# jstac/sdfs_via_autodiff

Hardware: AMD Instinct MI355X
Metric: fixed-point iterations/sec (higher is better)
Workload: dtype f64

## Files before the change

include/sdfs_hip.h:

```cpp
#ifndef SDFS_HIP_H
#define SDFS_HIP_H

#include <stdint.h>

#ifdef __cplusplus
extern "C" {
#endif

typedef struct sdfs_handle sdfs_handle;

enum { SDFS_MODEL_SSY = 0, SDFS_MODEL_GCY = 1 };
enum { SDFS_ALGO_SA = 0, SDFS_ALGO_NEWTON = 1, SDFS_ALGO_ANDERSON = 2 };

enum {
  SDFS_OK = 0,
  SDFS_ERR_ARG = -1,
  SDFS_ERR_HIP = -2,
  SDFS_ERR_UNSUPPORTED = -3,
  SDFS_ERR_NUMERIC = -4
};

typedef struct sdfs_opts {
  double tol;
  int64_t max_iter;
// ... 136 lines not shown
int sdfs_set_t_f32(sdfs_handle* h, int on, double w_ref);

int sdfs_set_profiling(sdfs_handle* h, int on);
int sdfs_reset_counters(sdfs_handle* h);
int sdfs_get_counters(sdfs_handle* h, sdfs_counters* out);

int sdfs_debug_pow(const double* x_host, double y, double* out_host, int64_t n, int device_id);
int sdfs_debug_powy(const double* x_host, double y, double* out_host, int64_t n, int degree, int device_id);
int sdfs_debug_jvp_storage_dev(sdfs_handle* h, int krylov_f32, const double* w_dev, const void* v_dev, void* out_dev,
                               int minus_identity);

int sdfs_stream_copy_dev(sdfs_handle* h, const double* src_dev, double* dst_dev, int64_t n);

int sdfs_describe_plan(const sdfs_handle* h, char* buf, int64_t cap);

typedef struct sdfs_batch sdfs_batch;

enum { SDFS_BATCH_CONVERGED = 0, SDFS_BATCH_MAX_ITER = 1, SDFS_BATCH_NONFINITE = 2 };

int64_t sdfs_batch_lds_bytes(int model, int ndim, const int64_t* shapes);

int sdfs_batch_create(int model, int ndim, const int64_t* shapes, int64_t B, const double* params,
                      const double* const* arrays, const int64_t* array_sizes, int narrays, int device_id,
                      sdfs_batch** out);
void sdfs_batch_destroy(sdfs_batch* h);
const char* sdfs_batch_last_error(const sdfs_batch* h);
int sdfs_batch_set_stream(sdfs_batch* h, void* hip_stream, int use_own);
int sdfs_batch_synchronize(sdfs_batch* h);

int sdfs_batch_apply_T_dev(sdfs_batch* h, const double* w_dev, double* Tw_dev, double* resid_dev);
// ... 14 lines not shown
```

sdfs_via_autodiff_amd/_lib.py:

```python
import ctypes as C
import os

_HERE = os.path.dirname(os.path.abspath(__file__))
LIB_PATH = os.path.join(_HERE, os.environ.get("SDFS_LIB_NAME", "libsdfs_hip.so"))

SDFS_MODEL_SSY, SDFS_MODEL_GCY = 0, 1
SDFS_ALGO_SA, SDFS_ALGO_NEWTON, SDFS_ALGO_ANDERSON = 0, 1, 2
SDFS_ERR_ARG = -1
SDFS_ERR_UNSUPPORTED = -3
SDFS_ERR_NUMERIC = -4
SDFS_MAX_KERNELS = 16
SDFS_BATCH_CONVERGED, SDFS_BATCH_MAX_ITER, SDFS_BATCH_NONFINITE = 0, 1, 2


class SdfsError(RuntimeError):
    pass


class sdfs_opts(C.Structure):
    _fields_ = [("tol", C.c_double), ("max_iter", C.c_int64),
                ("inner_rtol", C.c_double), ("inner_atol", C.c_double),
                ("inner_max_iter", C.c_int64),
                ("history", C.c_int32), ("mixing_freq", C.c_int32),
                ("beta", C.c_double), ("ridge", C.c_double),
# ... 66 lines not shown
    "sdfs_unpack_blocks_sub": (C.c_int, [_P, _P, _P, _P, C.c_int64, C.c_int64, C.c_int64, C.c_int, C.POINTER(C.c_int64), C.c_int]),
    "sdfs_anderson_begin": (C.c_int, [_P, C.c_int64, C.c_int, _P, _P, C.c_double, C.c_int64, C.c_double, C.c_double, C.c_int]),
    "sdfs_anderson_gate": (C.c_int, [_P, C.POINTER(_P)]),
    "sdfs_anderson_step": (C.c_int, [_P, C.c_int, C.c_int64, _P, _P, _P]),
    "sdfs_anderson_state": (C.c_int, [_P, _P, _P, C.c_int64, C.c_int64]),
    "sdfs_set_krylov_f32": (C.c_int, [_P, C.c_int, C.c_double]),
    "sdfs_set_t_f32": (C.c_int, [_P, C.c_int, C.c_double]),
    "sdfs_set_profiling": (C.c_int, [_P, C.c_int]),
    "sdfs_reset_counters": (C.c_int, [_P]),
    "sdfs_get_counters": (C.c_int, [_P, C.POINTER(sdfs_counters)]),
    "sdfs_describe_plan": (C.c_int, [_P, C.c_char_p, C.c_int64]),
    "sdfs_stream_copy_dev": (C.c_int, [_P, _P, _P, C.c_int64]),
    "sdfs_debug_pow": (C.c_int, [_P, C.c_double, _P, C.c_int64, C.c_int]),
    "sdfs_debug_powy": (C.c_int, [_P, C.c_double, _P, C.c_int64, C.c_int, C.c_int]),
    "sdfs_debug_jvp_storage_dev": (C.c_int, [_P, C.c_int, _P, _P, _P, C.c_int]),
    "sdfs_batch_lds_bytes": (C.c_int64, [C.c_int, C.c_int, _I64]),
    "sdfs_batch_create": (C.c_int, [C.c_int, C.c_int, _I64, C.c_int64, _D, C.POINTER(_D), _I64, C.c_int, C.c_int,
                                    C.POINTER(_P)]),
    "sdfs_batch_destroy": (None, [_P]),
    "sdfs_batch_last_error": (C.c_char_p, [_P]),
    "sdfs_batch_set_stream": (C.c_int, [_P, _P, C.c_int]),
    "sdfs_batch_synchronize": (C.c_int, [_P]),
    "sdfs_batch_apply_T_dev": (C.c_int, [_P, _P, _P, _P]),
    "sdfs_batch_solve_dev": (C.c_int, [_P, C.POINTER(sdfs_opts), _P, _I64, _D, C.POINTER(C.c_int32)]),
    "sdfs_batch_newton_dev": (C.c_int, [_P, C.POINTER(sdfs_opts), _P, _I64, _I64, _D, C.POINTER(C.c_int32)]),
    "sdfs_batch_describe": (C.c_int, [_P, C.c_char_p, C.c_int64]),
}


def _load():
# ... 35 lines not shown
```

sdfs_via_autodiff_amd/csrc/f32_kernels.hpp:

```cpp
#pragma once
#include "fast_kernels.hpp"

namespace sdfs {

typedef float v4f __attribute__((ext_vector_type(4)));
typedef float v2f __attribute__((ext_vector_type(2)));

template <int N> struct MShape32 {
  static_assert(N == 16 || N == 20 || N == 24 || N == 32, "pair plan extents");
  static constexpr int NT = (N + 15) / 16;
  static constexpr int KT = N / 4;
};

template <int N> struct QFrag32 {
  float a[MShape32<N>::NT][MShape32<N>::KT];
  __device__ __forceinline__ void load(const double* __restrict__ Q, int lane) {
    using S = MShape32<N>;
    const int li = lane & 15, lk = lane >> 4;
#pragma unroll
    for (int t = 0; t < S::NT; ++t) {
      const int row = 16 * t + li;
#pragma unroll
      for (int kk = 0; kk < S::KT; ++kk) a[t][kk] = row < N ? (float)Q[(row < N ? row : 0) * N + 4 * kk + lk] : 0.f;
    }
  }
};

template <int N, int RS>
__device__ __forceinline__ void ctile32(float* __restrict__ col, const int lk, const QFrag32<N>& q) {
  using S = MShape32<N>;
  float b[S::KT];
  const float* const pr = col + lk * RS;
#pragma unroll
  for (int kk = 0; kk < S::KT; ++kk) b[kk] = pr[4 * kk * RS];
  v4f acc[S::NT];
#pragma unroll
  for (int t = 0; t < S::NT; ++t) acc[t] = (v4f){0.f, 0.f, 0.f, 0.f};
#pragma unroll
  for (int kk = 0; kk < S::KT; ++kk) {
// ... 275 lines not shown
```

sdfs_via_autodiff_amd/csrc/fast_kernels.hpp:

```cpp
#pragma once
#include <hip/hip_runtime.h>
#include <stdint.h>

#include <type_traits>

#include "anderson_step.hpp"
#include "pass_kernel.hpp"
#include "wave_reduce.hpp"

namespace sdfs {

enum SliceMode { S_TFIRST = 0, S_TFIRST_LIN = 1, S_JFIRST = 2, S_MID = 3, S_TFIRST32 = 4, S_NMODES = 5 };
enum LineMode { L_MID = 0, L_TLAST = 1, L_TLAST_LIN = 2, L_JLAST = 3, L_TFUSED = 4, L_NMODES = 5 };

template <int N> struct MShape {
  static_assert(N == 16 || N == 20 || N == 24 || N == 32, "pair plan extents");
  static constexpr int N16 = N == 32 ? 2 : 1;
  static constexpr int N4 = (N - 16 * N16) / 4;
  static constexpr int KT = N / 4;
  static constexpr int A16 = N16, A4 = N4 > 0 ? N4 : 1;
};

template <int N> struct QFrag {
  double a16[MShape<N>::A16][MShape<N>::KT];
  double a4[MShape<N>::A4][MShape<N>::KT];
  __device__ __forceinline__ void load(const double* __restrict__ Q, int lane) {
    using S = MShape<N>;
    const int li = lane & 15, lk = lane >> 4, l4 = lane & 3;
#pragma unroll
    for (int kk = 0; kk < S::KT; ++kk) {
#pragma unroll
      for (int t = 0; t < S::N16; ++t) a16[t][kk] = Q[(16 * t + li) * N + 4 * kk + lk];
#pragma unroll
      for (int t = 0; t < S::N4; ++t) a4[t][kk] = Q[(16 * S::N16 + 4 * t + l4) * N + 4 * kk + lk];
    }
  }
};

template <int N, int RS>
__device__ __forceinline__ void ctile(double* __restrict__ p, const QFrag<N>& q) {
  using S = MShape<N>;
  double b[S::KT];
#pragma unroll
  for (int kk = 0; kk < S::KT; ++kk) b[kk] = p[4 * kk * RS];
  v4d acc[S::A16];
  double d[S::A4];
#pragma unroll
  for (int t = 0; t < S::A16; ++t) acc[t] = (v4d){0.0, 0.0, 0.0, 0.0};
#pragma unroll
// ... 91 lines not shown
template <int N, int WV = 4, bool PAD20 = false, int GX = 0> struct SliceGeo {
  static constexpr int G = GX > 0 ? GX : (N == 32 ? 2 : (N == 24 ? 2 : 4));
  static constexpr int RS = (N == 20 && !PAD20) ? N : N + 2;
  static constexpr int LTILE = G * N * RS;
  static constexpr int TILE = G * N * N;
  static constexpr int UNITS = TILE / 2;
  static constexpr int EPT = (UNITS + 63) / 64;
  static constexpr int NCT = (G * N + 15) / 16;
  static constexpr int CPAD = NCT * 16 - G * N;
  static constexpr int WAVES = WV;
  static constexpr int UNITS4 = TILE / 4;
  static constexpr int EPT4 = (UNITS4 + 63) / 64;
  static_assert(CPAD <= 8, "the repeated columns lie inside the last column tile");
};

template <int N, int MODE, bool F32, int WV = 4, bool PAD20 = false, int GX = 0, int OCC = 3>
__global__ void __launch_bounds__(64 * WV, OCC)
slice_kernel(const SliceDesc P, const SliceIO io) {
  using Geo = SliceGeo<N, WV, PAD20, GX>;
  constexpr bool T32 = MODE == S_TFIRST32;
  constexpr bool POWP = MODE == S_TFIRST || MODE == S_TFIRST_LIN || T32;
  constexpr bool LIN = MODE == S_TFIRST_LIN;
  constexpr bool MULP = MODE == S_JFIRST;
  constexpr bool JV32 = F32 && MULP;
  static_assert(!T32 || !F32, "S_TFIRST32 is its own storage form");
  constexpr bool POWREG = MODE == S_TFIRST || T32;
  static_assert(!F32 || (MODE != S_TFIRST && MODE != S_MID), "plain T has no fp32 form");
  extern __shared__ double lds[];
  if (io.gate != nullptr) {
    const unsigned long long g = *io.gate;
    if (g <= (unsigned long long)__double_as_longlong(io.gate_tol)) return;
  }
  const int lane = threadIdx.x & 63;
  const int wave = __builtin_amdgcn_readfirstlane(threadIdx.x >> 6);
  if (io.zero != nullptr && blockIdx.x == 0 && threadIdx.x == 0) *io.zero = 0ULL;
  const long long tile = (long long)blockIdx.x * Geo::WAVES + wave;
  const long long s0 = tile * Geo::G;
  if (s0 >= P.nslices) return;
  const long long rem = (P.nslices - s0) * (N * N / 2);
  const int nvalid = rem < Geo::UNITS ? (int)rem : Geo::UNITS;
  double* const wl = lds + wave * Geo::LTILE;
  auto lofs = [](const int e) -> int { return Geo::RS == N ? e : (e / N) * Geo::RS + (e % N); };
  const long long gbase = s0 * (N * N);
  const unsigned lb = (unsigned)lane * 16u;

  if (JV32) {
    const int nvalid4 = nvalid / 2;
    const char* const inb = reinterpret_cast<const char*>(reinterpret_cast<const float*>(io.in) + gbase);
    const char* const auxb = reinterpret_cast<const char*>(reinterpret_cast<const float*>(io.aux_in) + gbase);
    float4 v[Geo::EPT4], c1v[Geo::EPT4];
#pragma unroll
    for (int k = 0; k < Geo::EPT4; ++k) {
      const int u = lane + 64 * k;
      if (u < nvalid4) {
        v[k] = *reinterpret_cast<const float4*>(inb + (lb + 1024u * k));
        c1v[k] = *reinterpret_cast<const float4*>(auxb + (lb + 1024u * k));
      } else {
        v[k] = make_float4(0.f, 0.f, 0.f, 0.f); c1v[k] = v[k];
      }
    }
#pragma unroll
    for (int k = 0; k < Geo::EPT4; ++k) {
      const int u = lane + 64 * k;
      if (Geo::UNITS4 % 64 == 0 || u < Geo::UNITS4) {
        *reinterpret_cast<double2*>(wl + lofs(4 * u)) = make_double2((double)v[k].x * (double)c1v[k].x, (double)v[k].y * (double)c1v[k].y);
        *reinterpret_cast<double2*>(wl + lofs(4 * u + 2)) = make_double2((double)v[k].z * (double)c1v[k].z, (double)v[k].w * (double)c1v[k].w);
      }
    }
  } else {
    const char* const inb = reinterpret_cast<const char*>(io.in + gbase);
    const char* const auxb = reinterpret_cast<const char*>(io.aux_in + gbase);
    double2 v[Geo::EPT];
    double2 c1v[MULP ? Geo::EPT : 1];
#pragma unroll
    for (int k = 0; k < Geo::EPT; ++k) {
      const int u = lane + 64 * k;
      if (u < nvalid) {
        v[k] = ldg_stream2(inb + (lb + 1024u * k));
        if (MULP) c1v[MULP ? k : 0] = ldg_stream2(auxb + (lb + 1024u * k));
      } else {
        v[k] = make_double2(1.0, 1.0);
        if (MULP) c1v[MULP ? k : 0] = make_double2(0.0, 0.0);
      }
    }
    PowK<true> PTr;
    if (POWREG) PTr.init(P.theta, lane);
    double t32s = 1.0;
    if (T32) { const PowLane PL0 = pow_lane_init(lane); t32s = t32_scale_of(P.t32_ref > 0.0 ? P.t32_ref : io.in[P.ref_off], P.theta, PL0, false); }
#pragma unroll
    for (int k = 0; k < Geo::EPT; ++k) {
      const int u = lane + 64 * k;
      if (MULP) { v[k].x *= c1v[MULP ? k : 0].x; v[k].y *= c1v[MULP ? k : 0].y; }
      if (POWREG) {
        const double xin[2] = {v[k].x, v[k].y};
        double xw[2];
        PTr.template run<2>(xin, xw);
        v[k] = T32 ? make_double2(xw[0] * t32s, xw[1] * t32s) : make_double2(xw[0], xw[1]);
      }
      if (Geo::UNITS % 64 == 0 || u < Geo::UNITS) *reinterpret_cast<double2*>(wl + lofs(2 * u)) = v[k];
    }
  }
  QFrag<N> qf;
  qf.load(P.Qf, lane);
  wave_lds_fence();
  if (POWP && !POWREG) {
    const PowLane PT = pow_lane_init(lane);
    double lin_scale = 1.0;
    if (LIN && F32) lin_scale = lin_scale_of(io.in[P.ref_off], P.theta, PT, false);
    const double t32_scale = T32 ? t32_scale_of(P.t32_ref > 0.0 ? P.t32_ref : io.in[P.ref_off], P.theta, PT, false) : 1.0;
    char* const auxo = LIN ? (F32 ? reinterpret_cast<char*>(reinterpret_cast<float*>(io.aux_out) + gbase)
                                  : reinterpret_cast<char*>(io.aux_out + gbase)) : nullptr;
#pragma unroll 1
    for (int k = 0; k < Geo::EPT; ++k) {
      const int u = lane + 64 * k;
      const bool in_tile = Geo::UNITS % 64 == 0 || u < Geo::UNITS;
      const int lo = in_tile ? lofs(2 * u) : 0;
      const double2 x2 = *reinterpret_cast<const double2*>(wl + lo);
      const double xin[2] = {in_tile ? x2.x : 1.0, in_tile ? x2.y : 1.0};
      double xw[2];
// ... 8 lines not shown
      }
    }
    wave_lds_fence();
  }

  const int li = lane & 15, lk = lane >> 4;
  {
    double* const p0 = wl + li * Geo::RS + lk;
#pragma unroll
    for (int ct = 0; ct < Geo::NCT; ++ct) {
      const bool rep = Geo::CPAD > 0 && ct == Geo::NCT - 1;
      ctile<N, 1>(p0 + (ct * 16 - ((rep && li >= 16 - Geo::CPAD) ? Geo::CPAD : 0)) * Geo::RS, qf);
    }
  }
  wave_lds_fence();
  {
    QFrag<N> qe;
    qe.load(P.Qe, lane);
#pragma unroll
    for (int ct = 0; ct < Geo::NCT; ++ct) {
      const bool rep = Geo::CPAD > 0 && ct == Geo::NCT - 1;
      const int c = 16 * ct + li - ((rep && li >= 16 - Geo::CPAD) ? Geo::CPAD : 0);
      const int g = c / N, f = c - g * N;
      ctile<N, Geo::RS>(wl + g * (N * Geo::RS) + f + lk * Geo::RS, qe);
    }
  }
  wave_lds_fence();
  if (JV32 || T32) {
    const int nvalid4 = nvalid / 2;
    char* const outb = reinterpret_cast<char*>(reinterpret_cast<float*>(io.out) + gbase);
#pragma unroll
    for (int k = 0; k < Geo::EPT4; ++k) {
      const int u = lane + 64 * k;
      if (u < nvalid4) {
        const double2 a = *reinterpret_cast<const double2*>(wl + lofs(4 * u)), b = *reinterpret_cast<const double2*>(wl + lofs(4 * u + 2));
        *reinterpret_cast<float4*>(outb + (lb + 1024u * k)) = make_float4((float)a.x, (float)a.y, (float)b.x, (float)b.y);
      }
    }
  } else {
    char* const outb = reinterpret_cast<char*>(io.out + gbase);
#pragma unroll
    for (int k = 0; k < Geo::EPT; ++k) {
// ... 1053 lines not shown
```

sdfs_via_autodiff_amd/csrc/pad_kernels.hpp:

```cpp
#pragma once
#include <hip/hip_runtime.h>
#include <stdint.h>

#include "fast_kernels.hpp"

#ifndef SDFS_PAD_SOCC16
#define SDFS_PAD_SOCC16 3
#endif
#ifndef SDFS_PAD_SOCC24
#define SDFS_PAD_SOCC24 3
#endif
#ifndef SDFS_PAD_SOCC32
#define SDFS_PAD_SOCC32 3
#endif
#ifndef SDFS_PAD_SOCC16_J
#define SDFS_PAD_SOCC16_J 3
#endif
#ifndef SDFS_PAD_LOCC_MID16
#define SDFS_PAD_LOCC_MID16 3
#endif
#ifndef SDFS_PAD_LOCC_MID24
#define SDFS_PAD_LOCC_MID24 3
#endif
#ifndef SDFS_PAD_LOCC_MID32
// ... 79 lines not shown
      if (MULP) c1v[MULP ? k : 0] = e < nval ? io.aux_in[gbase + e] : 0.0;
    }
  }
#pragma unroll
  for (int k = 0; k < (PAD_LT + 63) / 64; ++k)
    if (PAD_LT % 64 == 0 || lane + 64 * k < PAD_LT) wl[lane + 64 * k] = 0.0;
  int lo[PAD_EPL];
#pragma unroll
  for (int k = 0; k < PAD_EPL; ++k) {
    const unsigned e = (unsigned)EI(k);
    const unsigned s = (e * P.mxy) >> 20, r = e - s * (unsigned)nxy;
    const unsigned x = (r * P.my) >> 20, y = r - x * (unsigned)P.ny;
    lo[k] = (int)((s * (unsigned)NT + x) * (unsigned)PAD_RS + y);
  }
  QFrag<NT> qf;
  qf.load(P.Qy, lane);
  wave_lds_fence();
  if (POWP) {
    PowK<true> PT;
    PT.init(P.theta, lane);
#pragma unroll
    for (int k = 0; k < PAD_EPL; k += 2) {
      if (NT == 32 && (PAIR ? 128 * (k >> 1) : 64 * k) >= nval) break;
      const double xin[2] = {v[k], v[k + 1]};
      double xw[2];
      PT.template run<2>(xin, xw);
      if (LIN) {
        if (PAIR) {
          if (EI(k) < nval) *reinterpret_cast<v2d*>(io.aux_out + gbase + EI(k)) = (v2d){xw[0] / xin[0], xw[1] / xin[1]};
        } else {
          if (EI(k) < nval) io.aux_out[gbase + EI(k)] = xw[0] / xin[0];
// ... 7 lines not shown
  for (int k = 0; k < PAD_EPL; ++k) {
    if (MULP) v[k] *= c1v[MULP ? k : 0];
    if (EI(k) < nval) wl[lo[k]] = v[k];
  }
  wave_lds_fence();
  const int li = lane & 15, lk = lane >> 4;
  constexpr int NCT = PAD_G * NT / 16;
  {
    double* const p0 = wl + li * PAD_RS + lk;
#pragma unroll
    for (int ct = 0; ct < NCT; ++ct) ctile<NT, 1>(p0 + ct * 16 * PAD_RS, qf);
  }
  wave_lds_fence();
  {
    QFrag<NT> qe;
    qe.load(P.Qx, lane);
#pragma unroll
    for (int ct = 0; ct < NCT; ++ct) {
      const int c = 16 * ct + li;
      const int g = c / NT, f = c - g * NT;
      ctile<NT, PAD_RS>(wl + g * (NT * PAD_RS) + f + lk * PAD_RS, qe);
    }
  }
  wave_lds_fence();
  if (PAIR) {
#pragma unroll
    for (int k = 0; k < PAD_EPL; k += 2)
      if (EI(k) < nval) *reinterpret_cast<v2d*>(io.out + gbase + EI(k)) = (v2d){wl[lo[k]], wl[lo[k + 1]]};
  } else {
#pragma unroll
    for (int k = 0; k < PAD_EPL; ++k)
// ... 64 lines not shown
  {
    double2 v[EPT];
#pragma unroll
    for (int k = 0; k < EPT; ++k) {
      int x, y; bool rok; long long off;
      unit_of(k, x, y, rok, off);
      v[k] = ld2(inb + off, pk0 && rok, pk1 && rok);
      if ((CES || MULE) && need_old) s1[(CES || MULE) ? k : 0] = ld2(oldb + off, pk0 && rok, pk1 && rok);
    }
#pragma unroll
    for (int k = 0; k < EPT; ++k)
      if (!Geo::PARTIAL || tid + B * k < Geo::UNITS) *reinterpret_cast<double2*>(lds + 2 * (tid + B * k)) = v[k];
  }
  {
    QFrag<NT> q;
    q.load(P.Qx, lane);
    __syncthreads();
    {
      double* const p0 = lds + li + lk * Geo::LX;
#pragma unroll
      for (int j = 0; j < (Geo::NCT + Geo::W - 1) / Geo::W; ++j)
        if (Geo::NCT % Geo::W == 0 || wave + j * Geo::W < Geo::NCT) ctile<NT, Geo::LX>(p0 + (wave + j * Geo::W) * 16, q);
    }
    q.load(P.Qy, lane);
    __syncthreads();
    {
      constexpr int XPT = 16 / R;
      double* const p0 = lds + (li / R) * Geo::LX + (li % R) + lk * R;
#pragma unroll
      for (int j = 0; j < (Geo::NCT + Geo::W - 1) / Geo::W; ++j)
        if (Geo::NCT % Geo::W == 0 || wave + j * Geo::W < Geo::NCT) ctile<NT, R>(p0 + (wave + j * Geo::W) * XPT * Geo::LX, q);
    }
    __syncthreads();
  }
  double* const outb = io.out + tbase;
  double rmax = 0.0, dot_yv = 0.0, dot_yy = 0.0;
  bool rnan = false;
  if (CES) {
    PowK<false> PT;
// ... 120 lines not shown
```

sdfs_via_autodiff_amd/csrc/sdfs_api.hip:

```cpp
#include <hip/hip_runtime.h>

#include <algorithm>
#include <cmath>
#include <cstdarg>
#include <cstdio>
#include <cstdlib>
#include <cstring>
#include <limits>
#include <map>
#include <mutex>
#include <string>
#include <type_traits>
#include <vector>

#include "../../include/sdfs_hip.h"
#include "pass_kernel.hpp"
#include "fast_kernels.hpp"
#include "stream_kernels.hpp"
#include "f32_kernels.hpp"
#include "pad_kernels.hpp"
#include "cont_kernel.hpp"
#include "dense_kernel.hpp"
#include "vec_kernels.hpp"
#include "krylov_kernels.hpp"
// ... 6 lines not shown
using namespace sdfs;

namespace {

constexpr int MAXD = 6;
constexpr int SCHED_WORDS = TK_WORDS;

thread_local std::string g_create_error;

struct AxisInfo {
  int n = 1;
  int nloc = 1;
  int off = 0;
  const double* Q = nullptr;
  const double* Qt = nullptr;
  const double* Qp = nullptr;
  const double* Qtp = nullptr;
  const double* Qpad[4] = {nullptr, nullptr, nullptr, nullptr};
  const double* Qtpad[4] = {nullptr, nullptr, nullptr, nullptr};
  int qs[MAXD] = {0, 0, 0, 0, 0, 0};
  long long qcount = 0;
  int a3s = 0;
  char name[8] = "";
};

struct Pass {
  PassDesc d;
  int block = 256;
  bool vec2 = false;
  bool vec4 = false;
// ... 683 lines not shown

std::vector<int> pair_order(int D) {
  std::vector<int> pairs = {D - 2};
  for (int a = 0; a <= D - 4; a += 2) pairs.push_back(a);
  return pairs;
}

void make_slice_pass(sdfs_handle* h, const int* shp, FastPass& P) {
  const int D = h->ndim;
  long long stride[MAXD], nloc = 1;
  for (int a = D - 1; a >= 0; --a) { stride[a] = nloc; nloc *= shp[a]; }
  const int n = shp[D - 1];
  P.line = false; P.n = n; P.ax0 = D - 2; P.ax1 = D - 1;
  memset(&P.sd, 0, sizeof P.sd);
  P.sd.nslices = nloc / ((long long)n * n);
  P.sd.Qf = h->ax[D - 1].Q; P.sd.Qe = h->ax[D - 2].Q; P.sd.theta = h->theta;
  for (int c = D - 1; c >= 0; --c) P.sd.ref_off += (long long)(shp[c] / 2) * stride[c];
  P.q_bytes = 2 * 8.0 * n * n; P.flops = 2.0 * (double)nloc * 2 * n;
  P.label = std::string("slices[") + h->ax[D - 2].name + "," + h->ax[D - 1].name + "|wave-private " +
            std::to_string(slice_tile_slices(n, S_TFIRST)) + "x" + std::to_string(n) + "x" + std::to_string(n) + "]";
}

int make_line_pass(sdfs_handle* h, const int* shp, const int* off, int a, bool tables, FastPass& P) {
  const int D = h->ndim;
  long long stride[MAXD], nloc = 1;
  for (int c = D - 1; c >= 0; --c) { stride[c] = nloc; nloc *= shp[c]; }
  const int n = shp[a];
  P.line = true; P.n = n; P.ax0 = a; P.ax1 = a + 1;
  memset(&P.ld, 0, sizeof P.ld);
  LineDesc& L = P.ld;
  L.lrest = stride[a + 1];
  if (L.lrest % 2 != 0) return 1;
  L.nchunks = (int)((L.lrest + LINE_R - 1) / LINE_R);
  L.nouter = nloc / ((long long)n * n * L.lrest);
  L.ntiles = L.nouter * L.nchunks;
  if (L.ntiles >= (1LL << 31) || (long long)n * n * L.lrest * 8 >= (1LL << 32)) return 1;
  L.Qx = h->ax[a].Q; L.Qy = h->ax[a + 1].Q;
  L.inv_theta = 1.0 / h->theta; L.beta = h->beta; L.theta = h->theta;
  L.cbt = (double)powl((long double)h->beta, (long double)h->theta);
  L.a3x = h->ax[a].a3s; L.a3y = h->ax[a + 1].a3s;
  for (int c = D - 1; c >= 0; --c) L.ref_off += (long long)(shp[c] / 2) * stride[c];
  L.cached_out = 8.0 * (double)nloc <= 192.0 * 1024 * 1024 ? 1 : 0;
  P.q_bytes = 2 * 8.0 * n * n; P.flops = 2.0 * (double)nloc * 2 * n;
  P.label = std::string("lines[") + h->ax[a].name + "," + h->ax[a + 1].name + "|" + std::to_string(n) + "x" +
            std::to_string(n) + "x16 tile]";
  if (!tables) return 0;
  std::vector<int> outv, restv;
  int *od = nullptr, *rd = nullptr;
  int rc;
  if ((rc = a3_index_tables(h, shp, off, a, outv, restv, &od, &rd))) return rc;
  L.a3 = h->a3; L.out_idx = od; L.rest_idx = rd;
  if (!h->a3_host.empty() && h->ax[a + 1].a3s == 0 && L.lrest % LINE_R == 0) {
// ... 487 lines not shown
        if (last) last_io(io);
        rc = launch_kernel(h, L.fn, L.grid, L.block, L.lds, d, io, L.tag, P.label, L.bytes, P.flops);
      }
    } else if (P.small) {
      SmallIO io;
      memset(&io, 0, sizeof io);
      io.in = pin; io.out = pout; io.gate = a.gate; io.gate_tol = a.gate_tol;
      SmallDesc d = P.sm;
      d.minus_identity = a.minus_identity;
      if (vjp) { d.Qxp = h->ax[P.ax0].Qtp; d.Qyp = h->ax[P.ax1].Qtp; }
      if (i == 0) first_io(io);
      else if (last) { last_io(io); io.dot_with = L.dot_with; }
      rc = launch_kernel(h, L.fn, L.grid, L.block, L.lds, d, io, L.tag, P.label, L.bytes, P.flops);
    } else if (!P.line) {
      SliceDesc sd = P.sd;
      if (vjp) { sd.Qf = h->ax[P.ax1].Qt; sd.Qe = h->ax[P.ax0].Qt; }
      if (h->sharded) sd.t32_ref = h->t32_ref;
      if (L.jfused && L.m32) {
        JFused32IO jio;
        memset(&jio, 0, sizeof jio);
        jio.upd = (float*)a.bicg.upd; jio.a = (const float*)a.bicg.a; jio.q = (const float*)a.bicg.q; jio.c1 = (const float*)h->c1;
        jio.out = (float*)pout; jio.sc = h->sc; jio.dot = a.bicg.dot; jio.gate = a.gate;
        rc = launch_kernel(h, L.fn, L.grid, L.block, L.lds, sd, jio, L.tag, P.label, L.bytes, P.flops);
      } else if (L.jfused) {
        JFusedIO jio;
        memset(&jio, 0, sizeof jio);
        jio.upd = a.bicg.upd; jio.a = a.bicg.a; jio.q = a.bicg.q; jio.c1 = h->c1; jio.out = pout; jio.sc = h->sc;
        jio.dot = a.bicg.dot; jio.gate = a.gate;
        rc = launch_kernel(h, L.fn, L.grid, L.block, L.lds, sd, jio, L.tag, P.label, L.bytes, P.flops);
      } else {
        SliceIO io;
        memset(&io, 0, sizeof io);
        io.in = pin; io.out = pout; io.gate = a.gate; io.gate_tol = a.gate_tol;
        first_io(io);
        rc = launch_kernel(h, L.fn, L.grid, L.block, L.lds, sd, io, L.tag, P.label, L.bytes, P.flops);
      }
    } else {
      LineIO io;
      memset(&io, 0, sizeof io);
      io.in = pin; io.out = pout; io.gate = a.gate; io.gate_tol = a.gate_tol;
      io.sched = h->sched + SCHED_WORDS * i;
      LineDesc d = P.ld;
      d.minus_identity = a.minus_identity;
      if (h->sharded) d.t32_ref = h->t32_ref;
      if (vjp) { d.Qx = h->ax[P.ax0].Qt; d.Qy = h->ax[P.ax1].Qt; }
      if (last) last_io(io);
      io.dot_with = L.dot_with;
      if (L.push) {
        io.and_y = a.push.y; io.and_r = a.push.r; io.and_beta = a.push.beta; io.and_dot = a.push.dot;
        if (a.push.tiles) *a.push.tiles = P.ld.ntiles;
      }
      rc = launch_kernel(h, L.fn, L.grid, L.block, L.lds, d, io, L.tag, P.label, L.bytes, P.flops);
    }
    if (rc) return rc;
    if (bf16) {
      if (mode == MODE_JVP && (rc = round_stream_bf16_n(h, pout, (long long)h->N, a.gate))) return rc;
      if (mode == MODE_T_LIN && i == 0 && (rc = round_stream_bf16_n(h, h->c1, (long long)h->N, nullptr))) return rc;
      if (mode == MODE_T_LIN && last && (rc = round_stream_bf16_n(h, h->c2, (long long)h->N, nullptr))) return rc;
    }
  }
// ... 1109 lines not shown
    hipDeviceProp_t prop;
    if (hipGetDeviceProperties(&prop, device_id) == hipSuccess && prop.multiProcessorCount > 0) h->num_cus = prop.multiProcessorCount;
  }
  int rc = setup_model(h, model, ndim, shapes, params, nparams, arrays, sizes, narrays);
  if (rc) return bail(rc);
  for (int a = 0; a < ndim; ++a) {
    if (h->ax[a].qcount != 1) continue;
    const int n = h->ax[a].n;
    std::vector<double> q((size_t)n * n), qt((size_t)n * n);
    if (hipMemcpy(q.data(), h->ax[a].Q, q.size() * sizeof(double), hipMemcpyDeviceToHost) != hipSuccess)
      return bail(fail(h, SDFS_ERR_HIP, "read-back of a transition matrix failed"));
    for (int i = 0; i < n; ++i) for (int j = 0; j < n; ++j) qt[(size_t)j * n + i] = q[(size_t)i * n + j];
    double* d = nullptr;
    if ((rc = upload(h, &d, qt.data(), qt.size()))) return bail(rc);
    h->ax[a].Qt = d;
    if (n <= 16) {
      std::vector<double> qp(256, 0.0), qtp(256, 0.0);
      for (int i = 0; i < n; ++i) for (int j = 0; j < n; ++j) { qp[(size_t)i * 16 + j] = q[(size_t)i * n + j]; qtp[(size_t)j * 16 + i] = q[(size_t)i * n + j]; }
      double *dp = nullptr, *dtp = nullptr;
      if ((rc = upload(h, &dp, qp.data(), 256)) || (rc = upload(h, &dtp, qtp.data(), 256))) return bail(rc);
      h->ax[a].Qp = dp; h->ax[a].Qtp = dtp;
    }
    for (int c = 0; c < 4; ++c) {
      const int nt = c == 0 ? 16 : (c == 1 ? 20 : (c == 2 ? 24 : 32));
      if (n > nt) continue;
      if (c == 0) { h->ax[a].Qpad[0] = h->ax[a].Qp; h->ax[a].Qtpad[0] = h->ax[a].Qtp; continue; }
      std::vector<double> qp((size_t)nt * nt, 0.0), qtp((size_t)nt * nt, 0.0);
      for (int i = 0; i < n; ++i) for (int j = 0; j < n; ++j) { qp[(size_t)i * nt + j] = q[(size_t)i * n + j]; qtp[(size_t)j * nt + i] = q[(size_t)i * n + j]; }
      double *dp = nullptr, *dtp = nullptr;
      if ((rc = upload(h, &dp, qp.data(), qp.size())) || (rc = upload(h, &dtp, qtp.data(), qtp.size()))) return bail(rc);
      h->ax[a].Qpad[c] = dp; h->ax[a].Qtpad[c] = dtp;
    }
  }
  static unsigned long long attr_done = 0;
  if (device_id < 64 && !(attr_done & (1ULL << device_id))) {
    for (int e = 1; e <= 16; e <<= 1)
      for (int v = 1; v <= 2; ++v)
        for (int j = 0; j < M_NMODES; ++j)
          for (int pr = 0; pr < 2; ++pr) {
            if (v == 2 && pr == 1) {
              pass_fn f4 = pass_kernel_variant(e, 4, j, 1);
// ... 1486 lines not shown
      BHIPCHK(h, hipFuncSetAttribute((const void*)h->nfn, hipFuncAttributeMaxDynamicSharedMemorySize, (int)h->lds_bytes));
      have = h->lds_bytes;
    }
  }
  const int slots = batch_newton_slots(h);
  if (!h->nst) BHIPCHK(h, hipMalloc((void**)&h->nst, (size_t)h->B * sizeof(BatchNewtonState)));
  BHIPCHK(h, hipMalloc((void**)&h->ws, (size_t)slots * BATCH_NEWTON_VECS * h->d.nwork * 8));
  h->ws_slots = slots;
  return 0;
}

}

extern "C" {

int64_t sdfs_batch_lds_bytes(int model, int ndim, const int64_t* shapes) {
  BatchDesc d;
  long long lds = 0;
  std::string why;
  const int rc = batch_geometry(model, ndim, shapes, d, &lds, &why);
  if (rc) { g_create_error = why; return rc; }
  return lds;
}

void sdfs_batch_destroy(sdfs_batch* h) {
  if (!h) return;
  hipSetDevice(h->device);
  if (h->stream) hipStreamSynchronize(h->stream);
  if (h->tab) hipFree(h->tab);
  if (h->d_dev) hipFree(h->d_dev);
// ... 220 lines not shown
```

sdfs_via_autodiff_amd/csrc/stream_kernels.hpp:

```cpp
#pragma once
#include "fast_kernels.hpp"

#ifndef SDFS_STREAM_STAMP
#define SDFS_STREAM_STAMP(i)
#define SDFS_STREAM_STAMP_NEXT
#define SDFS_STREAM_STAMP_DECL
#endif

#ifndef SDFS_LAST_SB
#define SDFS_LAST_SB 1
#endif

namespace sdfs {


constexpr unsigned NO_TILE = 0xffffffffu;
constexpr int TK_SUB = 4;
constexpr int TK_STRIDE = 16;
constexpr int TK_WORDS = (8 * TK_SUB + 1) * TK_STRIDE;
struct TicketWalk {
  unsigned start, count;
  unsigned* ctr;
  __device__ __forceinline__ TicketWalk(long long nunits, unsigned block, unsigned* sched) {
    const unsigned q = (unsigned)(nunits >> 3), r = (unsigned)(nunits & 7);
// ... 133 lines not shown
      wave_lds_fence();
#pragma unroll
      for (int k = 0; k < Geo::EPT; ++k) {
        const int u = lane + 64 * k;
        if (Geo::UNITS % 64 == 0 || u < Geo::UNITS) stg_stream<NT_SLICE>(outb + (lb + 1024u * k), *reinterpret_cast<const v2d*>(wl + lofs(2 * u)));
        if (k % 4 == 3) __builtin_amdgcn_sched_barrier(0);
      }
      wave_lds_fence();
      if (nxt == NO_TILE) break;
      cur = nxt; nxt = nn;
    }
  }
  if (lane == 0) ticket_walk_done(io.sched, gridDim.x * Geo::WAVES);
}

template <int N, int MODE, int WPC, bool OLDPF = false, int B = LineGeo<N>::B, bool PERSIST = true, bool A3F = false, bool IN32 = false,
          bool OUT32 = false, bool EARLY = false>
__global__ void __launch_bounds__(B, WPC * B / 256)
line_stream_kernel(const LineDesc P, const LineIO io) {
  using Geo = LineGeo<N>;
  static_assert(!EARLY || (OLDPF && !PERSIST && MODE == L_TLAST), "side stream with the tile: the one-tile-per-workgroup last pass of a plain T");
  constexpr int NW = B / 64;
  constexpr int EPT = (Geo::UNITS + B - 1) / B;
  constexpr bool CES = MODE == L_TLAST || MODE == L_TLAST_LIN;
  constexpr bool LINE = MODE == L_TLAST_LIN;
  constexpr bool MULE = MODE == L_JLAST;
  constexpr bool PARTIAL = Geo::UNITS % B != 0;
  constexpr int WHO = MODE == L_MID ? NT_MID : NT_LAST;
  static_assert(MODE != L_TFUSED, "the fused end + start form stays with line_kernel");
  static_assert(!OUT32 || MODE == L_MID, "fp32 output: the middle pass");
// ... 18 lines not shown
  const bool need_old = EARLY || (CES ? (io.resid != nullptr || andp) : (MULE && P.minus_identity));
  const char* const a3b = reinterpret_cast<const char*>(P.a3);
  const unsigned a3x = (unsigned)P.a3x, a3y = (unsigned)P.a3y;
  const TicketWalk W(P.ntiles, blockIdx.x, io.sched);
  __shared__ unsigned tk[3];
  unsigned cur, nxt = NO_TILE;
  int par = 0;
  if (PERSIST) {
    if (tid == 0) { const unsigned t0 = W.draw(); tk[0] = t0; tk[1] = t0 != NO_TILE ? W.draw() : NO_TILE; }
    __syncthreads();
    cur = tk[0]; nxt = tk[1];
    __syncthreads();
  } else {
    cur = (unsigned)xcd_remap((long long)blockIdx.x, P.ntiles);
  }
  QFrag<N> qx, qy_;
  qx.load(P.Qx, lane);
  if (PERSIST) qy_.load(P.Qy, lane);
  QFrag<N>& qy = PERSIST ? qy_ : qx;
  PowK<false> PT;
  if (CES) PT.init(P.inv_theta, lane);
  SDFS_STREAM_STAMP_DECL;
  double rmax = 0.0, dot_yv = 0.0, dot_yy = 0.0, dot_yr = 0.0;
  bool rnan = false;
  const bool dot3 = MULE && io.dot_with != nullptr;

  v2d v[IN32 ? 1 : EPT];
  float4 vf[IN32 ? EPT4 : 1];
  const unsigned e0 = (unsigned)(tid >> 2) * (unsigned)P.lrest + 4u * (tid & 3);
  const unsigned estep = (unsigned)(B / 4) * (unsigned)P.lrest;
  auto load32 = [&](const long long base) {
    const char* const inb = reinterpret_cast<const char*>(reinterpret_cast<const float*>(io.in) + base);
#pragma unroll
    for (int k = 0; k < EPT4; ++k) {
// ... 26 lines not shown
      if constexpr (IN32) {
#pragma unroll
        for (int k = 0; k < EPT4; ++k) {
          const int u = tid + k * B;
          if (!PART4 || u < Geo::UNITS4) {
            const float4 f = vf[IN32 ? k : 0];
            *reinterpret_cast<v2d*>(lds + 4 * u) = (v2d){(double)f.x * unscale32, (double)f.y * unscale32};
            *reinterpret_cast<v2d*>(lds + 4 * u + 2) = (v2d){(double)f.z * unscale32, (double)f.w * unscale32};
          }
        }
      } else {
#pragma unroll
        for (int k = 0; k < EPT; ++k)
          if (!PARTIAL || tid + k * B < Geo::UNITS) *reinterpret_cast<v2d*>(lds + 2 * (tid + k * B)) = v[k];
      }
      const bool has_next = PERSIST && nxt != NO_TILE;
      unsigned o; int chunk;
      const long long tbase = line_tile_base(P, cur, N * N, o, chunk);
      v2d f2v = (v2d){1.0, 1.0};
      if constexpr (A3F && EARLY) {
        if (tid < N) sF1[32 * par + tid] = f1e;
        f2v = f2e;
      } else if constexpr (A3F) {
        if (tid < N) sF1[32 * par + tid] = P.f1[(long long)o * N + tid];
        f2v = *reinterpret_cast<const v2d*>(P.f2 + (long long)o * P.lrest + (long long)chunk * LINE_R + 2 * c2);
      }
      if constexpr (OLDPF && !EARLY) { if (need_old) line_tile_load<EPT, B, Geo::UNITS, WHO>(wv, io.old + tbase, tid, b0, bstep); }
      unsigned o1; int ch1;
      const long long nbase = line_tile_base(P, has_next ? nxt : cur, N * N, o1, ch1);
      if (has_next) {
        if constexpr (IN32) load32(nbase);
        else line_tile_load<EPT, B, Geo::UNITS, WHO>(v, io.in + nbase, tid, b0, bstep);
      }
      unsigned nn = NO_TILE;
      if (PERSIST && tid == 0 && has_next) nn = W.draw();
      SDFS_STREAM_STAMP(1);
      __syncthreads();
      SDFS_STREAM_STAMP(2);
      {
        double* const p0 = lds + li + lk * Geo::LX;
#pragma unroll
        for (int j = 0; j < (N + NW - 1) / NW; ++j) { if (N % NW == 0 || wave + j * NW < N) ctile<N, Geo::LX>(p0 + (wave + j * NW) * 16, qx); __builtin_amdgcn_sched_barrier(0); }
      }
      SDFS_STREAM_STAMP(3);
      if (!PERSIST) qx.load(P.Qy, lane);
      __syncthreads();
      SDFS_STREAM_STAMP(4);
      {
        double* const p0 = lds + li + lk * LINE_R;
#pragma unroll
        for (int j = 0; j < (N + NW - 1) / NW; ++j) { if (N % NW == 0 || wave + j * NW < N) ctile<N, LINE_R>(p0 + (wave + j * NW) * Geo::LX, qy); __builtin_amdgcn_sched_barrier(0); }
      }
      SDFS_STREAM_STAMP(5);
      if (PERSIST && tid == 0) tk[par] = nn;
      __syncthreads();
      SDFS_STREAM_STAMP(6);
      char* const outb = reinterpret_cast<char*>(io.out + tbase);
      if constexpr (OUT32) {
        char* const outb4 = reinterpret_cast<char*>(reinterpret_cast<float*>(io.out) + tbase);
#pragma unroll
        for (int k = 0; k < EPT4; ++k) {
// ... 373 lines not shown
```

Measured before the change: 1389.

## Pre-swizzle Q fragment tables and issue Q loads earlier in slice/line kernels

Adds host-built per-lane fragment tables for the Q matrices, so each lane loads its MFMA operand fragments with coalesced double2/float4 reads instead of strided gathers. The slice kernel now starts the pow setup first and issues the Q loads earlier, overlapping them with the LDS staging. The non-persistent line kernel can keep Qy in a second register set, loaded up front or after the LDS park. This costs extra registers and device memory for the tables and adds compile-time switches, and the padded-path kernels move to the old gather loader.

```diff
diff --git a/include/sdfs_hip.h b/include/sdfs_hip.h
--- a/include/sdfs_hip.h
+++ b/include/sdfs_hip.h
@@ -174,6 +174,8 @@
 
 int sdfs_describe_plan(const sdfs_handle* h, char* buf, int64_t cap);
 
+int64_t sdfs_qfrag_table(int n, const double* Q, double* F, int64_t cap);
+
 typedef struct sdfs_batch sdfs_batch;
 
 enum { SDFS_BATCH_CONVERGED = 0, SDFS_BATCH_MAX_ITER = 1, SDFS_BATCH_NONFINITE = 2 };
diff --git a/sdfs_via_autodiff_amd/_lib.py b/sdfs_via_autodiff_amd/_lib.py
--- a/sdfs_via_autodiff_amd/_lib.py
+++ b/sdfs_via_autodiff_amd/_lib.py
@@ -104,6 +104,7 @@
     "sdfs_debug_pow": (C.c_int, [_P, C.c_double, _P, C.c_int64, C.c_int]),
     "sdfs_debug_powy": (C.c_int, [_P, C.c_double, _P, C.c_int64, C.c_int, C.c_int]),
     "sdfs_debug_jvp_storage_dev": (C.c_int, [_P, C.c_int, _P, _P, _P, C.c_int]),
+    "sdfs_qfrag_table": (C.c_int64, [C.c_int, _D, _D, C.c_int64]),
     "sdfs_batch_lds_bytes": (C.c_int64, [C.c_int, C.c_int, _I64]),
     "sdfs_batch_create": (C.c_int, [C.c_int, C.c_int, _I64, C.c_int64, _D, C.POINTER(_D), _I64, C.c_int, C.c_int,
                                     C.POINTER(_P)]),
diff --git a/sdfs_via_autodiff_amd/csrc/f32_kernels.hpp b/sdfs_via_autodiff_amd/csrc/f32_kernels.hpp
--- a/sdfs_via_autodiff_amd/csrc/f32_kernels.hpp
+++ b/sdfs_via_autodiff_amd/csrc/f32_kernels.hpp
@@ -14,8 +14,11 @@
 
 template <int N> struct QFrag32 {
   float a[MShape32<N>::NT][MShape32<N>::KT];
-  __device__ __forceinline__ void load(const double* __restrict__ Q, int lane) {
+  static constexpr int FROW = (MShape32<N>::NT * MShape32<N>::KT + 3) & ~3;
+  __device__ __forceinline__ void load(const double* __restrict__ F, int lane) {
     using S = MShape32<N>;
+#if SDFS_QFRAG_GATHER
+    const double* __restrict__ Q = F;
     const int li = lane & 15, lk = lane >> 4;
 #pragma unroll
     for (int t = 0; t < S::NT; ++t) {
@@ -23,6 +26,21 @@
 #pragma unroll
       for (int kk = 0; kk < S::KT; ++kk) a[t][kk] = row < N ? (float)Q[(row < N ? row : 0) * N + 4 * kk + lk] : 0.f;
     }
+#else
+    const float4* __restrict__ const r = reinterpret_cast<const float4*>(F + 64 * QFrag<N>::FROW) + lane;
+    float4 u[FROW / 4];
+#pragma unroll
+    for (int i = 0; i < FROW / 4; ++i) u[i] = r[64 * i];
+#pragma unroll
+    for (int t = 0; t < S::NT; ++t) {
+#pragma unroll
+      for (int kk = 0; kk < S::KT; ++kk) {
+        const int j = t * S::KT + kk;
+        const float4 q = u[j >> 2];
+        a[t][kk] = (j & 3) == 0 ? q.x : ((j & 3) == 1 ? q.y : ((j & 3) == 2 ? q.z : q.w));
+      }
+    }
+#endif
   }
 };
 
diff --git a/sdfs_via_autodiff_amd/csrc/fast_kernels.hpp b/sdfs_via_autodiff_amd/csrc/fast_kernels.hpp
--- a/sdfs_via_autodiff_amd/csrc/fast_kernels.hpp
+++ b/sdfs_via_autodiff_amd/csrc/fast_kernels.hpp
@@ -21,10 +21,48 @@
   static constexpr int A16 = N16, A4 = N4 > 0 ? N4 : 1;
 };
 
+#ifndef SDFS_QFRAG_GATHER
+#define SDFS_QFRAG_GATHER 0
+#endif
+
+inline int qfrag_row_doubles(int n) {
+  const int n16 = n == 32 ? 2 : 1, n4 = (n - 16 * n16) / 4;
+  return ((n / 4) * (n16 + n4) + 1) & ~1;
+}
+inline int qfrag_row_floats(int n) { return (((n + 15) / 16) * (n / 4) + 3) & ~3; }
+inline size_t qfrag_table_doubles(int n) {
+  return SDFS_QFRAG_GATHER ? (size_t)n * n : (size_t)64 * qfrag_row_doubles(n) + (size_t)32 * qfrag_row_floats(n);
+}
+inline void qfrag_table_fill(const double* Q, int n, double* F) {
+  if (SDFS_QFRAG_GATHER) { for (int i = 0; i < n * n; ++i) F[i] = Q[i]; return; }
+  {
+    float* const G = reinterpret_cast<float*>(F + (size_t)64 * qfrag_row_doubles(n));
+    const int nt = (n + 15) / 16, kt = n / 4, row = qfrag_row_floats(n);
+    for (int l = 0; l < 64; ++l) {
+      int j = 0;
+      auto put = [&](float x) { G[(size_t)(j >> 2) * 256 + 4 * l + (j & 3)] = x; ++j; };
+      for (int t = 0; t < nt; ++t) for (int kk = 0; kk < kt; ++kk) {
+        const int r = 16 * t + (l & 15);
+        put(r < n ? (float)Q[(size_t)r * n + 4 * kk + (l >> 4)] : 0.f);
+      }
+      while (j < row) put(0.f);
+    }
+  }
+  const int n16 = n == 32 ? 2 : 1, n4 = (n - 16 * n16) / 4, kt = n / 4, row = qfrag_row_doubles(n);
+  for (int l = 0; l < 64; ++l) {
+    int j = 0;
+    auto put = [&](double x) { F[(size_t)(j >> 1) * 128 + 2 * l + (j & 1)] = x; ++j; };
+    for (int t = 0; t < n16; ++t) for (int kk = 0; kk < kt; ++kk) put(Q[(size_t)(16 * t + (l & 15)) * n + 4 * kk + (l >> 4)]);
+    for (int t = 0; t < n4; ++t) for (int kk = 0; kk < kt; ++kk) put(Q[(size_t)(16 * n16 + 4 * t + (l & 3)) * n + 4 * kk + (l >> 4)]);
+    while (j < row) put(0.0);
+  }
+}
+
 template <int N> struct QFrag {
   double a16[MShape<N>::A16][MShape<N>::KT];
   double a4[MShape<N>::A4][MShape<N>::KT];
-  __device__ __forceinline__ void load(const double* __restrict__ Q, int lane) {
+  static constexpr int FROW = (MShape<N>::KT * (MShape<N>::N16 + MShape<N>::N4) + 1) & ~1;
+  __device__ __forceinline__ void load_matrix(const double* __restrict__ Q, int lane) {
     using S = MShape<N>;
     const int li = lane & 15, lk = lane >> 4, l4 = lane & 3;
 #pragma unroll
@@ -33,6 +71,37 @@
       for (int t = 0; t < S::N16; ++t) a16[t][kk] = Q[(16 * t + li) * N + 4 * kk + lk];
 #pragma unroll
       for (int t = 0; t < S::N4; ++t) a4[t][kk] = Q[(16 * S::N16 + 4 * t + l4) * N + 4 * kk + lk];
+    }
+  }
+  __device__ __forceinline__ void load(const double* __restrict__ F, int lane) {
+    using S = MShape<N>;
+#if SDFS_QFRAG_GATHER
+    load_matrix(F, lane);
+#else
+    const double2* __restrict__ const r = reinterpret_cast<const double2*>(F) + lane;
+    double2 u[FROW / 2];
+#pragma unroll
+    for (int i = 0; i < FROW / 2; ++i) u[i] = r[64 * i];
+#pragma unroll
+    for (int t = 0; t < S::N16; ++t) {
+#pragma unroll
+      for (int kk = 0; kk < S::KT; ++kk) { const int j = t * S::KT + kk; a16[t][kk] = (j & 1) ? u[j >> 1].y : u[j >> 1].x; }
+    }
+#pragma unroll
+    for (int t = 0; t < S::N4; ++t) {
+#pragma unroll
+      for (int kk = 0; kk < S::KT; ++kk) { const int j = (S::N16 + t) * S::KT + kk; a4[t][kk] = (j & 1) ? u[j >> 1].y : u[j >> 1].x; }
+    }
+#endif
+  }
+  __device__ __forceinline__ void landed() {
+    using S = MShape<N>;
+#pragma unroll
+    for (int kk = 0; kk < S::KT; ++kk) {
+#pragma unroll
+      for (int t = 0; t < S::N16; ++t) asm volatile("" : "+v"(a16[t][kk]));
+#pragma unroll
+      for (int t = 0; t < S::N4; ++t) asm volatile("" : "+v"(a4[t][kk]));
     }
   }
 };
@@ -154,6 +223,16 @@
   static_assert(CPAD <= 8, "the repeated columns lie inside the last column tile");
 };
 
+#ifndef SDFS_SLICE_POW_FIRST
+#define SDFS_SLICE_POW_FIRST 1
+#endif
+#ifndef SDFS_SLICE_Q_EARLY
+#define SDFS_SLICE_Q_EARLY 1
+#endif
+#ifndef SDFS_SLICE_STAMP
+#define SDFS_SLICE_STAMP(i)
+#endif
+
 template <int N, int MODE, bool F32, int WV = 4, bool PAD20 = false, int GX = 0, int OCC = 3>
 __global__ void __launch_bounds__(64 * WV, OCC)
 slice_kernel(const SliceDesc P, const SliceIO io) {
@@ -165,6 +244,8 @@
   constexpr bool JV32 = F32 && MULP;
   static_assert(!T32 || !F32, "S_TFIRST32 is its own storage form");
   constexpr bool POWREG = MODE == S_TFIRST || T32;
+  constexpr bool POWFIRST = POWREG && SDFS_SLICE_POW_FIRST;
+  constexpr bool QEARLY = POWREG && SDFS_SLICE_Q_EARLY;
   static_assert(!F32 || (MODE != S_TFIRST && MODE != S_MID), "plain T has no fp32 form");
   extern __shared__ double lds[];
   if (io.gate != nullptr) {
@@ -183,6 +264,8 @@
   auto lofs = [](const int e) -> int { return Geo::RS == N ? e : (e / N) * Geo::RS + (e % N); };
   const long long gbase = s0 * (N * N);
   const unsigned lb = (unsigned)lane * 16u;
+  QFrag<N> qf, qe;
+  SDFS_SLICE_STAMP(0);
 
   if (JV32) {
     const int nvalid4 = nvalid / 2;
@@ -210,6 +293,8 @@
   } else {
     const char* const inb = reinterpret_cast<const char*>(io.in + gbase);
     const char* const auxb = reinterpret_cast<const char*>(io.aux_in + gbase);
+    PowK<true> PTr;
+    if (POWFIRST) { PTr.init(P.theta, lane); __builtin_amdgcn_sched_barrier(0); }
     double2 v[Geo::EPT];
     double2 c1v[MULP ? Geo::EPT : 1];
 #pragma unroll
@@ -223,13 +308,17 @@
         if (MULP) c1v[MULP ? k : 0] = make_double2(0.0, 0.0);
       }
     }
-    PowK<true> PTr;
-    if (POWREG) PTr.init(P.theta, lane);
+    if (POWREG && !POWFIRST) PTr.init(P.theta, lane);
     double t32s = 1.0;
     if (T32) { const PowLane PL0 = pow_lane_init(lane); t32s = t32_scale_of(P.t32_ref > 0.0 ? P.t32_ref : io.in[P.ref_off], P.theta, PL0, false); }
 #pragma unroll
     for (int k = 0; k < Geo::EPT; ++k) {
       const int u = lane + 64 * k;
+      if (QEARLY && k == (Geo::EPT > 3 ? Geo::EPT - 3 : 0)) {
+        __builtin_amdgcn_sched_barrier(0);
+        qf.load(P.Qf, lane);
+        __builtin_amdgcn_sched_barrier(0);
+      }
       if (MULP) { v[k].x *= c1v[MULP ? k : 0].x; v[k].y *= c1v[MULP ? k : 0].y; }
       if (POWREG) {
         const double xin[2] = {v[k].x, v[k].y};
@@ -240,9 +329,17 @@
       if (Geo::UNITS % 64 == 0 || u < Geo::UNITS) *reinterpret_cast<double2*>(wl + lofs(2 * u)) = v[k];
     }
   }
-  QFrag<N> qf;
-  qf.load(P.Qf, lane);
+  SDFS_SLICE_STAMP(1);
+  if (QEARLY) {
+    __builtin_amdgcn_sched_barrier(0);
+    qe.load(P.Qe, lane);
+    __builtin_amdgcn_sched_barrier(0);
+  } else {
+    qf.load(P.Qf, lane);
+  }
   wave_lds_fence();
+  qf.landed();
+  SDFS_SLICE_STAMP(2);
   if (POWP && !POWREG) {
     const PowLane PT = pow_lane_init(lane);
     double lin_scale = 1.0;
@@ -281,9 +378,11 @@
     }
   }
   wave_lds_fence();
+  SDFS_SLICE_STAMP(3);
   {
-    QFrag<N> qe;
-    qe.load(P.Qe, lane);
+    if (!QEARLY) qe.load(P.Qe, lane);
+    qe.landed();
+    SDFS_SLICE_STAMP(4);
 #pragma unroll
     for (int ct = 0; ct < Geo::NCT; ++ct) {
       const bool rep = Geo::CPAD > 0 && ct == Geo::NCT - 1;
@@ -293,6 +392,7 @@
     }
   }
   wave_lds_fence();
+  SDFS_SLICE_STAMP(5);
   if (JV32 || T32) {
     const int nvalid4 = nvalid / 2;
     char* const outb = reinterpret_cast<char*>(reinterpret_cast<float*>(io.out) + gbase);
diff --git a/sdfs_via_autodiff_amd/csrc/pad_kernels.hpp b/sdfs_via_autodiff_amd/csrc/pad_kernels.hpp
--- a/sdfs_via_autodiff_amd/csrc/pad_kernels.hpp
+++ b/sdfs_via_autodiff_amd/csrc/pad_kernels.hpp
@@ -117,7 +117,7 @@
     lo[k] = (int)((s * (unsigned)NT + x) * (unsigned)PAD_RS + y);
   }
   QFrag<NT> qf;
-  qf.load(P.Qy, lane);
+  qf.load_matrix(P.Qy, lane);
   wave_lds_fence();
   if (POWP) {
     PowK<true> PT;
@@ -155,7 +155,7 @@
   wave_lds_fence();
   {
     QFrag<NT> qe;
-    qe.load(P.Qx, lane);
+    qe.load_matrix(P.Qx, lane);
 #pragma unroll
     for (int ct = 0; ct < NCT; ++ct) {
       const int c = 16 * ct + li;
@@ -250,7 +250,7 @@
   }
   {
     QFrag<NT> q;
-    q.load(P.Qx, lane);
+    q.load_matrix(P.Qx, lane);
     __syncthreads();
     {
       double* const p0 = lds + li + lk * Geo::LX;
@@ -258,7 +258,7 @@
       for (int j = 0; j < (Geo::NCT + Geo::W - 1) / Geo::W; ++j)
         if (Geo::NCT % Geo::W == 0 || wave + j * Geo::W < Geo::NCT) ctile<NT, Geo::LX>(p0 + (wave + j * Geo::W) * 16, q);
     }
-    q.load(P.Qy, lane);
+    q.load_matrix(P.Qy, lane);
     __syncthreads();
     {
       constexpr int XPT = 16 / R;
diff --git a/sdfs_via_autodiff_amd/csrc/sdfs_api.hip b/sdfs_via_autodiff_amd/csrc/sdfs_api.hip
--- a/sdfs_via_autodiff_amd/csrc/sdfs_api.hip
+++ b/sdfs_via_autodiff_amd/csrc/sdfs_api.hip
@@ -44,6 +44,8 @@
   int off = 0;
   const double* Q = nullptr;
   const double* Qt = nullptr;
+  const double* Qfr = nullptr;
+  const double* Qtfr = nullptr;
   const double* Qp = nullptr;
   const double* Qtp = nullptr;
   const double* Qpad[4] = {nullptr, nullptr, nullptr, nullptr};
@@ -757,7 +759,7 @@
   P.line = false; P.n = n; P.ax0 = D - 2; P.ax1 = D - 1;
   memset(&P.sd, 0, sizeof P.sd);
   P.sd.nslices = nloc / ((long long)n * n);
-  P.sd.Qf = h->ax[D - 1].Q; P.sd.Qe = h->ax[D - 2].Q; P.sd.theta = h->theta;
+  P.sd.Qf = h->ax[D - 1].Qfr; P.sd.Qe = h->ax[D - 2].Qfr; P.sd.theta = h->theta;
   for (int c = D - 1; c >= 0; --c) P.sd.ref_off += (long long)(shp[c] / 2) * stride[c];
   P.q_bytes = 2 * 8.0 * n * n; P.flops = 2.0 * (double)nloc * 2 * n;
   P.label = std::string("slices[") + h->ax[D - 2].name + "," + h->ax[D - 1].name + "|wave-private " +
@@ -778,7 +780,7 @@
   L.nouter = nloc / ((long long)n * n * L.lrest);
   L.ntiles = L.nouter * L.nchunks;
   if (L.ntiles >= (1LL << 31) || (long long)n * n * L.lrest * 8 >= (1LL << 32)) return 1;
-  L.Qx = h->ax[a].Q; L.Qy = h->ax[a + 1].Q;
+  L.Qx = h->ax[a].Qfr; L.Qy = h->ax[a + 1].Qfr;
   L.inv_theta = 1.0 / h->theta; L.beta = h->beta; L.theta = h->theta;
   L.cbt = (double)powl((long double)h->beta, (long double)h->theta);
   L.a3x = h->ax[a].a3s; L.a3y = h->ax[a + 1].a3s;
@@ -1296,7 +1298,7 @@
       rc = launch_kernel(h, L.fn, L.grid, L.block, L.lds, d, io, L.tag, P.label, L.bytes, P.flops);
     } else if (!P.line) {
       SliceDesc sd = P.sd;
-      if (vjp) { sd.Qf = h->ax[P.ax1].Qt; sd.Qe = h->ax[P.ax0].Qt; }
+      if (vjp) { sd.Qf = h->ax[P.ax1].Qtfr; sd.Qe = h->ax[P.ax0].Qtfr; }
       if (h->sharded) sd.t32_ref = h->t32_ref;
       if (L.jfused && L.m32) {
         JFused32IO jio;
@@ -1325,7 +1327,7 @@
       LineDesc d = P.ld;
       d.minus_identity = a.minus_identity;
       if (h->sharded) d.t32_ref = h->t32_ref;
-      if (vjp) { d.Qx = h->ax[P.ax0].Qt; d.Qy = h->ax[P.ax1].Qt; }
+      if (vjp) { d.Qx = h->ax[P.ax0].Qtfr; d.Qy = h->ax[P.ax1].Qtfr; }
       if (last) last_io(io);
       io.dot_with = L.dot_with;
       if (L.push) {
@@ -2465,17 +2467,26 @@
     double* d = nullptr;
     if ((rc = upload(h, &d, qt.data(), qt.size()))) return bail(rc);
     h->ax[a].Qt = d;
+    auto upload_frag = [&](const std::vector<double>& m, int nt, double** out) -> int {
+      std::vector<double> f(qfrag_table_doubles(nt));
+      qfrag_table_fill(m.data(), nt, f.data());
+      return upload(h, out, f.data(), f.size());
+    };
+    if (n == 16 || n == 20 || n == 24 || n == 32) {
+      double *df = nullptr, *dtf = nullptr;
+      if ((rc = upload_frag(q, n, &df)) || (rc = upload_frag(qt, n, &dtf))) return bail(rc);
+      h->ax[a].Qfr = df; h->ax[a].Qtfr = dtf;
+    }
     if (n <= 16) {
       std::vector<double> qp(256, 0.0), qtp(256, 0.0);
       for (int i = 0; i < n; ++i) for (int j = 0; j < n; ++j) { qp[(size_t)i * 16 + j] = q[(size_t)i * n + j]; qtp[(size_t)j * 16 + i] = q[(size_t)i * n + j]; }
       double *dp = nullptr, *dtp = nullptr;
-      if ((rc = upload(h, &dp, qp.data(), 256)) || (rc = upload(h, &dtp, qtp.data(), 256))) return bail(rc);
+      if ((rc = upload_frag(qp, 16, &dp)) || (rc = upload_frag(qtp, 16, &dtp))) return bail(rc);
       h->ax[a].Qp = dp; h->ax[a].Qtp = dtp;
     }
     for (int c = 0; c < 4; ++c) {
       const int nt = c == 0 ? 16 : (c == 1 ? 20 : (c == 2 ? 24 : 32));
       if (n > nt) continue;
-      if (c == 0) { h->ax[a].Qpad[0] = h->ax[a].Qp; h->ax[a].Qtpad[0] = h->ax[a].Qtp; continue; }
       std::vector<double> qp((size_t)nt * nt, 0.0), qtp((size_t)nt * nt, 0.0);
       for (int i = 0; i < n; ++i) for (int j = 0; j < n; ++j) { qp[(size_t)i * nt + j] = q[(size_t)i * n + j]; qtp[(size_t)j * nt + i] = q[(size_t)i * n + j]; }
       double *dp = nullptr, *dtp = nullptr;
@@ -3992,6 +4003,15 @@
 
 extern "C" {
 
+int64_t sdfs_qfrag_table(int n, const double* Q, double* F, int64_t cap) {
+  if (!(n == 16 || n == 20 || n == 24 || n == 32)) return SDFS_ERR_ARG;
+  const int64_t need = (int64_t)qfrag_table_doubles(n);
+  if (F == nullptr) return need;
+  if (Q == nullptr || cap < need) return SDFS_ERR_ARG;
+  qfrag_table_fill(Q, n, F);
+  return need;
+}
+
 int64_t sdfs_batch_lds_bytes(int model, int ndim, const int64_t* shapes) {
   BatchDesc d;
   long long lds = 0;
diff --git a/sdfs_via_autodiff_amd/csrc/stream_kernels.hpp b/sdfs_via_autodiff_amd/csrc/stream_kernels.hpp
--- a/sdfs_via_autodiff_amd/csrc/stream_kernels.hpp
+++ b/sdfs_via_autodiff_amd/csrc/stream_kernels.hpp
@@ -171,6 +171,13 @@
   if (lane == 0) ticket_walk_done(io.sched, gridDim.x * Geo::WAVES);
 }
 
+#ifndef SDFS_LAST_QY_UPFRONT
+#define SDFS_LAST_QY_UPFRONT 1
+#endif
+template <int N, int MODE, bool A3F, bool IN32, bool EARLY> struct LastQy {
+  static constexpr bool UPFRONT = SDFS_LAST_QY_UPFRONT != 0 && (N == 16 || (N == 20 && !IN32 && !EARLY));
+  static constexpr bool AFTERPARK = SDFS_LAST_QY_UPFRONT != 0 && EARLY && !IN32 && !UPFRONT;
+};
 template <int N, int MODE, int WPC, bool OLDPF = false, int B = LineGeo<N>::B, bool PERSIST = true, bool A3F = false, bool IN32 = false,
           bool OUT32 = false, bool EARLY = false>
 __global__ void __launch_bounds__(B, WPC * B / 256)
@@ -219,10 +226,12 @@
   } else {
     cur = (unsigned)xcd_remap((long long)blockIdx.x, P.ntiles);
   }
+  constexpr bool QY2 = PERSIST || (OLDPF && LastQy<N, MODE, A3F, IN32, EARLY>::UPFRONT);
+  constexpr bool QYPARK = !PERSIST && OLDPF && LastQy<N, MODE, A3F, IN32, EARLY>::AFTERPARK;
   QFrag<N> qx, qy_;
   qx.load(P.Qx, lane);
-  if (PERSIST) qy_.load(P.Qy, lane);
-  QFrag<N>& qy = PERSIST ? qy_ : qx;
+  if (QY2) qy_.load(P.Qy, lane);
+  QFrag<N>& qy = (QY2 || QYPARK) ? qy_ : qx;
   PowK<false> PT;
   if (CES) PT.init(P.inv_theta, lane);
   SDFS_STREAM_STAMP_DECL;
@@ -279,6 +288,7 @@
         for (int k = 0; k < EPT; ++k)
           if (!PARTIAL || tid + k * B < Geo::UNITS) *reinterpret_cast<v2d*>(lds + 2 * (tid + k * B)) = v[k];
       }
+      if constexpr (QYPARK) { __builtin_amdgcn_sched_barrier(0); qy_.load(P.Qy, lane); __builtin_amdgcn_sched_barrier(0); }
       const bool has_next = PERSIST && nxt != NO_TILE;
       unsigned o; int chunk;
       const long long tbase = line_tile_base(P, cur, N * N, o, chunk);
@@ -301,6 +311,7 @@
       if (PERSIST && tid == 0 && has_next) nn = W.draw();
       SDFS_STREAM_STAMP(1);
       __syncthreads();
+      if (!PERSIST) qx.landed();
       SDFS_STREAM_STAMP(2);
       {
         double* const p0 = lds + li + lk * Geo::LX;
@@ -308,8 +319,9 @@
         for (int j = 0; j < (N + NW - 1) / NW; ++j) { if (N % NW == 0 || wave + j * NW < N) ctile<N, Geo::LX>(p0 + (wave + j * NW) * 16, qx); __builtin_amdgcn_sched_barrier(0); }
       }
       SDFS_STREAM_STAMP(3);
-      if (!PERSIST) qx.load(P.Qy, lane);
+      if (!QY2 && !QYPARK) qx.load(P.Qy, lane);
       __syncthreads();
+      if (!PERSIST) qy.landed();
       SDFS_STREAM_STAMP(4);
       {
         double* const p0 = lds + li + lk * LINE_R;
```

New measurement: 1398, median of 6. No clear change (+0.7%).
